# ypw0102/GDR

Measured on AMD Instinct MI355X. Metric: queries/sec on NQ-320k (768-d), higher is better.
Workload: dtype f32; 1 GPU; C2/ragged/prefilter: t5-base encoder 512 q/GPU + Q.D^T top-100, 320000x768 corpus; batch_per_gpu=512, global_batch=512, seq_len=40, corpus_rows=320000, dim=768, k=100, encoder_rows=ragged

## Files before the change

gdr_amd/csrc/sim_topk.hip:

```cpp
#include <stdlib.h>

#include "common.h"

namespace gdr {

constexpr int TILE = 128;
constexpr int SEL_THREADS = 256;

struct SimPlan {
  int64_t tiles_m;
  int stride;
  int64_t n_sample_tiles;
  int64_t n_slots;
  int64_t cap;
  size_t off_val, off_idx, off_cnt, off_thr, off_part, total;
};

static SimPlan make_plan(int B, int64_t N, int k, bool exhaustive, double survivors = 1.0) {
  SimPlan p{};
  p.tiles_m = (N + TILE - 1) / TILE;
  double target = sqrt((double)k * (double)N);
  if (target < k) target = k;
  int64_t ts = (int64_t)((target + TILE - 1) / TILE);
  if (ts < 1) ts = 1;
  if (exhaustive || N <= 16384 || p.tiles_m < 4 * ts) {
    p.stride = 1;
  } else {
    p.stride = (int)(p.tiles_m / ts);
  }
  p.n_sample_tiles = (p.tiles_m + p.stride - 1) / p.stride;
  p.n_slots = p.n_sample_tiles * TILE;
  if (p.stride == 1) {
    p.cap = p.n_slots;
  } else {
    const double n_sample = (double)p.n_slots;
    const double expect = (double)k * (double)N / n_sample;
    p.cap = p.n_slots + (int64_t)(4.0 * expect * survivors) + 4096;
    p.cap = (p.cap + TILE - 1) / TILE * TILE;
  }
  size_t o = 0;
  p.off_val = o, o += align_up((size_t)B * p.cap * sizeof(float), 256);
  p.off_idx = o, o += align_up((size_t)B * p.cap * sizeof(int32_t), 256);
  p.off_cnt = o, o += align_up((size_t)B * CNT_STRIDE * sizeof(int32_t), 256);
  p.off_thr = o, o += align_up((size_t)B * sizeof(float), 256);
  p.off_part = o, o += B <= 32 ? align_up((size_t)B * 16 * 128 * sizeof(unsigned long long), 256) : 0;
  p.total = o;
  return p;
}

__device__ __forceinline__ uint32_t fkey(float v) {
  const uint32_t u = __float_as_uint(v);
  return (u & 0x80000000u) ? ~u : (u | 0x80000000u);
}
__device__ __forceinline__ float fkey_inv(uint32_t k) {
  return __uint_as_float((k & 0x80000000u) ? (k & 0x7fffffffu) : ~k);
}

__device__ __forceinline__ int find_bin(int* hist, int* scan, int& need, int* above, int* res) {
  const int t = threadIdx.x, lane = t & 63, wave = t >> 6;
  const int v = t < 256 ? hist[t] : 0;
  int sfx = v;
#pragma unroll
  for (int off = 1; off < 64; off <<= 1) {
    const int u = __shfl_down(sfx, off);
    if (lane + off < 64) sfx += u;
  }
  if (t < 256 && lane == 0) scan[wave] = sfx;
  if (t == 0) res[0] = 0, res[1] = 0;
  __syncthreads();
  const int w0 = scan[0], w1 = scan[1], w2 = scan[2], w3 = scan[3];
  const int total = w0 + w1 + w2 + w3;
  if (total < need) need = total;
  if (t < 256 && need > 0) {
    const int higher = wave == 0 ? w1 + w2 + w3 : wave == 1 ? w2 + w3 : wave == 2 ? w3 : 0;
    const int mine = sfx + higher, next = mine - v;
    if (mine >= need && next < need) {
      res[0] = t;
      res[1] = next;
    }
  }
  __syncthreads();
  *above = res[1];
  return res[0];
}

__device__ __forceinline__ void wave0_bitonic_desc(unsigned long long* buf, int kpad) {
  if (threadIdx.x >= 64) return;
  const int lane = threadIdx.x;
  for (int size = 2; size <= kpad; size <<= 1) {
    for (int stride = size >> 1; stride > 0; stride >>= 1) {
      for (int t = lane; t < (kpad >> 1); t += 64) {
        const int lo_i = (t / stride) * (stride << 1) + (t % stride), hi_i = lo_i + stride;
        const bool desc = ((lo_i & size) == 0);
        const unsigned long long a = buf[lo_i], b = buf[hi_i];
        if ((a < b) == desc) buf[lo_i] = b, buf[hi_i] = a;
      }
      __builtin_amdgcn_fence(__ATOMIC_RELEASE, "wavefront");
      __builtin_amdgcn_wave_barrier();
      __builtin_amdgcn_fence(__ATOMIC_ACQUIRE, "wavefront");
    }
  }
}

__device__ __forceinline__ void block_minmax(uint32_t& lo, uint32_t& hi, uint32_t* red) {
#pragma unroll
  for (int off = 32; off > 0; off >>= 1) {
    lo = min(lo, (uint32_t)__shfl_xor((int)lo, off));
    hi = max(hi, (uint32_t)__shfl_xor((int)hi, off));
  }
  const int w = threadIdx.x >> 6, nw = blockDim.x >> 6;
  if ((threadIdx.x & 63) == 0) red[w] = lo, red[16 + w] = hi;
  __syncthreads();
  lo = red[0], hi = red[16];
  for (int i = 1; i < nw; ++i) lo = min(lo, red[i]), hi = max(hi, red[16 + i]);
  __syncthreads();
}


__global__ __launch_bounds__(1024) void sim_threshold_kernel(const float* __restrict__ cand_val, int64_t cap,
                                                             int n_slots, int k, float* thr, int32_t* cand_cnt,
                                                             const float* __restrict__ sub) {
  __shared__ int hist[256];
  __shared__ int scan[256];
  __shared__ int res[2];
  __shared__ uint32_t red[32];
  const int q = blockIdx.x;
  const float* v = cand_val + (int64_t)q * cap;
  constexpr int RC = 8;
  const bool cached = n_slots <= RC * (int)blockDim.x;
  uint32_t rk[RC];
#pragma unroll
  for (int u = 0; u < RC; ++u) {
    const int i = threadIdx.x + u * (int)blockDim.x;
    rk[u] = (cached && i < n_slots) ? fkey(v[i]) : 0u;
  }
  const uint32_t kneg = fkey(-INFINITY);
  uint32_t lo = 0xFFFFFFFFu, hi = 0u;
  if (cached) {
#pragma unroll
    for (int u = 0; u < RC; ++u)
      if (rk[u] > kneg) lo = min(lo, rk[u]), hi = max(hi, rk[u]);
  } else {
#pragma unroll 4
    for (int i = threadIdx.x; i < n_slots; i += blockDim.x) {
      const float x = v[i];
      if (x > -INFINITY) {
        const uint32_t key = fkey(x);
        lo = min(lo, key), hi = max(hi, key);
      }
    }
  }
  block_minmax(lo, hi, red);
  if (hi < lo) lo = hi = fkey(-INFINITY);
  const int nbits = hi > lo ? 32 - __clz(hi - lo) : 0;
  const int lsh = 32 - nbits;
  uint32_t prefix = 0;
  int need = k;
  for (int pass = 0; 8 * pass < nbits; ++pass) {
    const int shift = 24 - 8 * pass;
    if (threadIdx.x < 256) hist[threadIdx.x] = 0;
    __syncthreads();
    if (cached) {
#pragma unroll
      for (int u = 0; u < RC; ++u) {
        const uint32_t raw = rk[u];
        const uint32_t key = (raw - lo) << lsh;
        const bool match = pass == 0 ? true : ((key >> (shift + 8)) == (prefix >> (shift + 8)));
        if (raw != 0u && match && raw >= lo) atomicAdd(&hist[(key >> shift) & 255u], 1);
      }
    } else {
#pragma unroll 4
      for (int i = threadIdx.x; i < n_slots; i += blockDim.x) {
        const uint32_t raw = fkey(v[i]);
        const uint32_t key = (raw - lo) << lsh;
        const bool match = pass == 0 ? true : ((key >> (shift + 8)) == (prefix >> (shift + 8)));
        if (match && raw >= lo) atomicAdd(&hist[(key >> shift) & 255u], 1);
      }
    }
    __syncthreads();
    int above;
    const int b = find_bin(hist, scan, need, &above, res);
    need -= above;
    prefix |= (uint32_t)b << shift;
    __syncthreads();
  }
  if (threadIdx.x == 0) {
    const float t = fkey_inv(nbits ? (prefix >> lsh) + lo : lo);
    thr[q] = sub ? t - sub[q] : t;
    cand_cnt[(int64_t)q * CNT_STRIDE] = n_slots;
  }
}

template <bool MERGE>
__global__ __launch_bounds__(1024) void topk_select_kernel(const float* __restrict__ vals,
                                                           const int32_t* __restrict__ idxs,
                                                           const int32_t* __restrict__ cnt, int64_t cap, int G, int B,
                                                           int k, int kpad, int32_t idx_offset,
                                                           const float* __restrict__ thr, float* out_val,
                                                           int32_t* out_idx, int32_t* __restrict__ status, int rs,
                                                           int es) {
  __shared__ int hist[256];
  __shared__ int scan[256];
  __shared__ int res[2];
  __shared__ uint32_t red[32];
  __shared__ int n_out;
  extern __shared__ __attribute__((aligned(16))) unsigned long long sortbuf[];
  const int q = blockIdx.x;
  int count;
  if (MERGE) {
    count = G * k;
    if (status && rs > k && threadIdx.x == 0) {
      int32_t any = 0;
      for (int g = 0; g < G; ++g) any |= idxs[(((int64_t)g * B + q) * rs + k) * es];
      status[q] = any != 0 ? 1 : 0;
    }
  } else {
    const int c = cnt[(int64_t)q * CNT_STRIDE];
    count = c < (int)cap ? c : (int)cap;
    if (status && threadIdx.x == 0) status[q] = c > (int)cap ? 1 : 0;
  }
  auto addr_of = [&](int i) -> int64_t {
    if (MERGE) {
      const int g = i / k, j = i - g * k;
      return (((int64_t)g * B + q) * rs + j) * es;
    }
    return (int64_t)q * cap + i;
  };
  constexpr int RC = 16;
  const bool cached = count <= RC * (int)blockDim.x;
  auto raw_at = [&](int i) -> unsigned long long {
    const int64_t a = addr_of(i);
    const int32_t id = idxs[a];
    if (id < 0) return 0ull;
    return ((unsigned long long)fkey(vals[a]) << 32) | (unsigned long long)(0xFFFFFFFFu - (uint32_t)id);
  };
  unsigned long long rk[RC];
#pragma unroll
  for (int u = 0; u < RC; ++u) {
    const int i = threadIdx.x + u * (int)blockDim.x;
    rk[u] = (cached && i < count) ? raw_at(i) : 0ull;
  }
  uint32_t lo = 0xFFFFFFFFu, hi = 0u;
  if (cached) {
#pragma unroll
    for (int u = 0; u < RC; ++u)
      if (rk[u] != 0ull) {
        const uint32_t key = (uint32_t)(rk[u] >> 32);
        lo = min(lo, key), hi = max(hi, key);
      }
  } else {
#pragma unroll 4
    for (int i = threadIdx.x; i < count; i += blockDim.x) {
      const unsigned long long raw = raw_at(i);
      if (raw != 0ull) {
        const uint32_t key = (uint32_t)(raw >> 32);
        lo = min(lo, key), hi = max(hi, key);
      }
    }
  }
  block_minmax(lo, hi, red);
  if (!MERGE && thr) lo = max(lo, fkey(thr[q]));
  if (hi < lo) hi = lo;
  const int nbits = hi > lo ? 32 - __clz(hi - lo) : 0;
  const int lsh = 32 - nbits;
  auto norm = [&](unsigned long long raw) -> unsigned long long {
    if (raw == 0ull) return 0ull;
    const uint32_t sk = (uint32_t)(raw >> 32);
    if (sk < lo) return 0ull;
    return ((((unsigned long long)(sk - lo)) << 32) | (raw & 0xFFFFFFFFull)) << lsh;
  };
  unsigned long long prefix = 0ull;
  int need = k < count ? k : count;
  int want = need;
  bool exact = false;
  for (int pass = 0; pass < 8 && !exact; ++pass) {
    const int shift = 56 - 8 * pass;
    if (threadIdx.x < 256) hist[threadIdx.x] = 0;
    __syncthreads();
    if (cached) {
#pragma unroll
      for (int u = 0; u < RC; ++u) {
        const unsigned long long key = norm(rk[u]);
        const bool match = pass == 0 ? true : ((key >> (shift + 8)) == (prefix >> (shift + 8)));
        if (match && key != 0ull) atomicAdd(&hist[(int)((key >> shift) & 255ull)], 1);
      }
    } else {
#pragma unroll 4
      for (int i = threadIdx.x; i < count; i += blockDim.x) {
        const unsigned long long key = norm(raw_at(i));
        const bool match = pass == 0 ? true : ((key >> (shift + 8)) == (prefix >> (shift + 8)));
        if (match && key != 0ull) atomicAdd(&hist[(int)((key >> shift) & 255ull)], 1);
      }
    }
    __syncthreads();
    int above;
    const int b = find_bin(hist, scan, need, &above, res);
    if (pass == 0) want = need;
    need -= above;
    prefix |= (unsigned long long)b << shift;
    exact = hist[b] == need;
    __syncthreads();
  }
  if (threadIdx.x == 0) n_out = 0;
  for (int i = threadIdx.x; i < kpad; i += blockDim.x) sortbuf[i] = 0ull;
  __syncthreads();
  if (cached) {
#pragma unroll
    for (int u = 0; u < RC; ++u) {
      const unsigned long long key = norm(rk[u]);
      if (key >= prefix && key != 0ull) {
        const int p = atomicAdd(&n_out, 1);
        if (p < kpad) sortbuf[p] = rk[u];
      }
    }
  } else {
#pragma unroll 4
    for (int i = threadIdx.x; i < count; i += blockDim.x) {
      const unsigned long long raw = raw_at(i);
      const unsigned long long key = norm(raw);
      if (key >= prefix && key != 0ull) {
        const int p = atomicAdd(&n_out, 1);
        if (p < kpad) sortbuf[p] = raw;
      }
    }
  }
  __syncthreads();
  wave0_bitonic_desc(sortbuf, kpad);
  __syncthreads();
  for (int i = threadIdx.x; i < k; i += blockDim.x) {
    const unsigned long long key = sortbuf[i];
    float v = -INFINITY;
    int32_t id = -1;
    if (i < want && key != 0ull) {
      v = fkey_inv((uint32_t)(key >> 32));
      id = (int32_t)(0xFFFFFFFFu - (uint32_t)(key & 0xFFFFFFFFull)) + idx_offset;
    }
    out_val[(int64_t)q * k + i] = v;
    out_idx[(int64_t)q * k + i] = id;
  }
}

constexpr int SL_THREADS = 256, SL_RC = 8, SL_NS_MAX = 16, SL_KPAD_MAX = 128;
struct SelLds {
  int hist[256];
  int scan[256];
  int res[2];
  uint32_t red[32];
  int n_out, last;
};

template <int RC>
__device__ __forceinline__ int block_select_keys(const unsigned long long (&rk)[RC], int k, int kpad, uint32_t lo_floor, SelLds& L,
                                                 unsigned long long* outbuf) {
  uint32_t lo = 0xFFFFFFFFu, hi = 0u;
#pragma unroll
  for (int u = 0; u < RC; ++u)
    if (rk[u] != 0ull) {
      const uint32_t key = (uint32_t)(rk[u] >> 32);
      lo = min(lo, key), hi = max(hi, key);
    }
  block_minmax(lo, hi, L.red);
  lo = max(lo, lo_floor);
  if (hi < lo) hi = lo;
  const int nbits = hi > lo ? 32 - __clz(hi - lo) : 0;
  const int lsh = 32 - nbits;
  auto norm = [&](unsigned long long raw) -> unsigned long long {
    if (raw == 0ull) return 0ull;
    const uint32_t sk = (uint32_t)(raw >> 32);
    if (sk < lo) return 0ull;
    return ((((unsigned long long)(sk - lo)) << 32) | (raw & 0xFFFFFFFFull)) << lsh;
  };
  unsigned long long prefix = 0ull;
  int need = k, want = k;
  bool exact = false;
  for (int pass = 0; pass < 8 && !exact; ++pass) {
    const int shift = 56 - 8 * pass;
    L.hist[threadIdx.x] = 0;
    __syncthreads();
#pragma unroll
    for (int u = 0; u < RC; ++u) {
      const unsigned long long key = norm(rk[u]);
      const bool match = pass == 0 ? true : ((key >> (shift + 8)) == (prefix >> (shift + 8)));
      if (match && key != 0ull) atomicAdd(&L.hist[(int)((key >> shift) & 255ull)], 1);
    }
    __syncthreads();
    int above;
    const int b = find_bin(L.hist, L.scan, need, &above, L.res);
    if (pass == 0) want = need;
    need -= above;
    prefix |= (unsigned long long)b << shift;
    exact = L.hist[b] == need;
    __syncthreads();
  }
  if (threadIdx.x == 0) L.n_out = 0;
  for (int i = threadIdx.x; i < kpad; i += SL_THREADS) outbuf[i] = 0ull;
  __syncthreads();
  if (want > 0) {
#pragma unroll
    for (int u = 0; u < RC; ++u) {
      const unsigned long long key = norm(rk[u]);
      if (key >= prefix && key != 0ull) {
        const int p = atomicAdd(&L.n_out, 1);
        if (p < kpad) outbuf[p] = rk[u];
      }
    }
  }
  __syncthreads();
  return want;
}

struct SlicedArgs {
  const float* vals;
  const int32_t* idxs;
  int32_t* cnt;
  int64_t cap;
  int n_slots;
  int k, kpad, NS;
  int32_t idx_offset;
  float* thr;
  const float* sub;
  unsigned long long* part;
  float* out_val;
  int32_t* out_idx;
  int32_t* status;
};

template <bool THR>
__global__ __launch_bounds__(SL_THREADS) void sim_sliced_select_kernel(const SlicedArgs a) {
  __shared__ SelLds L;
  __shared__ __attribute__((aligned(16))) unsigned long long outbuf[SL_KPAD_MAX];
  const int q = blockIdx.x / a.NS, s = blockIdx.x % a.NS, tid = threadIdx.x;
  int count;
  if (THR) {
    count = a.n_slots;
  } else {
    const int c = a.cnt[(int64_t)q * CNT_STRIDE];
    count = c < (int)a.cap ? c : (int)a.cap;
  }
  const int per = (count + a.NS - 1) / a.NS;
  const int i0 = s * per, i1 = min(count, i0 + per);
  const float* v = a.vals + (int64_t)q * a.cap;
  const int32_t* ix = a.idxs + (int64_t)q * a.cap;
  unsigned long long rk[SL_RC];
#pragma unroll
  for (int u = 0; u < SL_RC; ++u) {
    const int i = i0 + tid + u * SL_THREADS;
    unsigned long long raw = 0ull;
    if (i < i1) {
      const float x = v[i];
      if (THR) {
        if (x > -INFINITY) raw = ((unsigned long long)fkey(x) << 32) | (unsigned long long)(0xFFFFFFFFu - (uint32_t)i);
      } else {
        const int32_t id = ix[i];
        if (id >= 0) raw = ((unsigned long long)fkey(x) << 32) | (unsigned long long)(0xFFFFFFFFu - (uint32_t)id);
      }
    }
    rk[u] = raw;
  }
  const uint32_t floor_key = (!THR && a.thr) ? fkey(a.thr[q]) : 0u;
  block_select_keys<SL_RC>(rk, a.k, a.kpad, floor_key, L, outbuf);
  unsigned long long* mine = a.part + ((int64_t)q * a.NS + s) * a.kpad;
  if (tid < a.kpad) {
    const unsigned long long key = outbuf[tid];
    typedef unsigned int u32x2 __attribute__((ext_vector_type(2)));
    u32x2 w;
    w[0] = (unsigned int)(key & 0xFFFFFFFFull), w[1] = (unsigned int)(key >> 32);
    const __amdgpu_buffer_rsrc_t dst = __builtin_amdgcn_make_buffer_rsrc(mine, 0, a.kpad * 8, 0x00020000);
    __builtin_amdgcn_raw_buffer_store_b64(w, dst, tid * 8, 0, 16);
  }
  asm volatile("s_waitcnt vmcnt(0)" ::: "memory");
  __syncthreads();
  int32_t* ticket = a.cnt + (int64_t)q * CNT_STRIDE + (THR ? 1 : 2);
  if (tid == 0) {
    const int t = __hip_atomic_fetch_add(ticket, 1, __ATOMIC_RELAXED, __HIP_MEMORY_SCOPE_AGENT);
    L.last = t == a.NS - 1;
    if (L.last) {
      __builtin_amdgcn_fence(__ATOMIC_ACQUIRE, "agent");
      asm volatile("s_waitcnt vmcnt(0)" ::: "memory");
    }
  }
  __syncthreads();
  if (!L.last) return;
  const unsigned long long* all = a.part + (int64_t)q * a.NS * a.kpad;
  const int n_all = a.NS * a.kpad;
#pragma unroll
  for (int u = 0; u < SL_RC; ++u) {
    const int i = tid + u * SL_THREADS;
    rk[u] = i < n_all ? all[i] : 0ull;
  }
  const int want = block_select_keys<SL_RC>(rk, a.k, a.kpad, 0u, L, outbuf);
  if (THR) {
    unsigned long long m = tid < want ? outbuf[tid] : ~0ull;
#pragma unroll
    for (int off = 32; off > 0; off >>= 1) {
      const unsigned long long o = __shfl_xor(m, off);
      m = o < m ? o : m;
    }
    if ((tid & 63) == 0) reinterpret_cast<unsigned long long*>(L.hist)[tid >> 6] = m;
    __syncthreads();
    if (tid == 0) {
      const unsigned long long* w4 = reinterpret_cast<const unsigned long long*>(L.hist);
      unsigned long long mm = w4[0];
      for (int i = 1; i < SL_THREADS / 64; ++i) mm = w4[i] < mm ? w4[i] : mm;
      const float t = want > 0 ? fkey_inv((uint32_t)(mm >> 32)) : -INFINITY;
      a.thr[q] = a.sub ? t - a.sub[q] : t;
      a.cnt[(int64_t)q * CNT_STRIDE] = a.n_slots;
      a.cnt[(int64_t)q * CNT_STRIDE + 1] = 0;
      a.cnt[(int64_t)q * CNT_STRIDE + 2] = 0;
    }
    return;
  }
  wave0_bitonic_desc(outbuf, a.kpad);
  __syncthreads();
  for (int i = tid; i < a.k; i += SL_THREADS) {
    const unsigned long long key = outbuf[i];
    float val = -INFINITY;
    int32_t id = -1;
    if (i < want && key != 0ull) {
      val = fkey_inv((uint32_t)(key >> 32));
      id = (int32_t)(0xFFFFFFFFu - (uint32_t)(key & 0xFFFFFFFFull)) + a.idx_offset;
    }
    a.out_val[(int64_t)q * a.k + i] = val;
    a.out_idx[(int64_t)q * a.k + i] = id;
  }
  if (tid == 0) {
    const int c = a.cnt[(int64_t)q * CNT_STRIDE];
    if (a.status) a.status[q] = c > (int)a.cap ? 1 : 0;
    a.cnt[(int64_t)q * CNT_STRIDE + 2] = 0;
  }
}

static int sliced_ns(int64_t len, int kpad) {
  if (kpad > SL_KPAD_MAX || len > (int64_t)SL_NS_MAX * SL_RC * SL_THREADS) return 0;
  int ns = (int)((len + 1023) / 1024);
  const int need = (int)((len + SL_RC * SL_THREADS - 1) / (SL_RC * SL_THREADS));
  if (ns < need) ns = need;
  if (ns < 1) ns = 1;
  if (ns > SL_NS_MAX) ns = SL_NS_MAX;
  while ((int64_t)ns * kpad > SL_RC * SL_THREADS) --ns;
  return ns >= need ? ns : 0;
}

static int next_pow2(int x) {
  int p = 1;
  while (p < x) p <<= 1;
  return p;
}

}

extern "C" size_t gdr_sim_topk_workspace_bytes(int B, int64_t N, int d, int k, int flags) {
  (void)d;
  if (B <= 0 || N <= 0 || k <= 0) return 0;
  return gdr::make_plan(B, N, k, (flags & GDR_SIM_EXHAUSTIVE) != 0).total;
}

namespace gdr {
__global__ __launch_bounds__(256) void cast_f32_bf16_kernel(const float4* __restrict__ in, uint2* __restrict__ out,
                                                            int64_t n4) {
  const int64_t i = (int64_t)blockIdx.x * 256 + threadIdx.x;
  if (i >= n4) return;
  const float4 v = in[i];
  union {
    __bf16 h[4];
    uint2 u;
  } o;
  o.h[0] = (__bf16)v.x, o.h[1] = (__bf16)v.y, o.h[2] = (__bf16)v.z, o.h[3] = (__bf16)v.w;
  out[i] = o.u;
}

static int sim_topk_impl(const void* Q, int B, const void* D, int64_t N, int d, int k, int32_t idx_offset, float* out_val,
                         int32_t* out_idx, int32_t* status, int flags, void* workspace, size_t workspace_bytes,
                         bool bf16, hipStream_t stream);
}

namespace gdr {
int launch_cast_f32_bf16(const float* in, void* out_bf16, int64_t n, hipStream_t stream) {
  if (n == 0) return GDR_OK;
  GDR_CHECK_ARG(in && out_bf16 && n >= 0 && n % 4 == 0, "cast: null pointer or n %% 4 != 0");
  GDR_CHECK_ARG(((uintptr_t)in & 15) == 0 && ((uintptr_t)out_bf16 & 7) == 0, "cast: misaligned pointer");
  if (n == 0) return GDR_OK;
  hipLaunchKernelGGL(cast_f32_bf16_kernel, dim3((unsigned)((n / 4 + 255) / 256)), dim3(256), 0, stream,
                     reinterpret_cast<const float4*>(in), reinterpret_cast<uint2*>(out_bf16), n / 4);
  GDR_CHECK_LAUNCH("cast_f32_bf16_kernel");
  return GDR_OK;
}
}

extern "C" int gdr_cast_f32_bf16(const float* in, void* out_bf16, int64_t n, void* stream_) {
  return gdr::launch_cast_f32_bf16(in, out_bf16, n, static_cast<hipStream_t>(stream_));
}

extern "C" int gdr_sim_topk(const float* Q, int B, const float* D, int64_t N, int d, int k, int32_t idx_offset,
                            float* out_val, int32_t* out_idx, int32_t* status, int flags, void* workspace,
                            size_t workspace_bytes, void* stream_) {
  return gdr::sim_topk_impl(Q, B, D, N, d, k, idx_offset, out_val, out_idx, status, flags, workspace, workspace_bytes,
                            false, static_cast<hipStream_t>(stream_));
}

extern "C" int gdr_sim_topk_bf16(const void* Q, int B, const void* D, int64_t N, int d, int k, int32_t idx_offset,
                                 float* out_val, int32_t* out_idx, int32_t* status, int flags, void* workspace,
                                 size_t workspace_bytes, void* stream_) {
  return gdr::sim_topk_impl(Q, B, D, N, d, k, idx_offset, out_val, out_idx, status, flags, workspace, workspace_bytes,
                            true, static_cast<hipStream_t>(stream_));
}

int gdr::sim_topk_impl(const void* Q, int B, const void* D, int64_t N, int d, int k, int32_t idx_offset,
                       float* out_val, int32_t* out_idx, int32_t* status, int flags, void* workspace,
                       size_t workspace_bytes, bool bf16, hipStream_t stream) {
  if (B == 0) return GDR_OK;
  GDR_CHECK_ARG(Q && D && out_val && out_idx && workspace, "sim_topk: null pointer");
  GDR_CHECK_ARG(B > 0 && N > 0 && d > 0 && d % (bf16 ? 8 : 4) == 0, "sim_topk: bad shape B=%d N=%lld d=%d", B,
                (long long)N, d);
  GDR_CHECK_ARG(k >= 1 && k <= 1024 && k <= N, "sim_topk: k=%d must be in [1, min(1024, N)]", k);
  GDR_CHECK_ARG(N < 0x7fffffffLL - 256, "sim_topk: shard too large for int32 doc ids");
  GDR_CHECK_ARG((int64_t)idx_offset + N <= 0x7fffffffLL,
                "sim_topk: idx_offset=%d + N=%lld leaves int32 doc ids (the largest id, idx_offset + N - 1, must be < 2^31 - 1)", (int)idx_offset,
                (long long)N);
  GDR_CHECK_ARG(((uintptr_t)Q & 15) == 0 && ((uintptr_t)D & 15) == 0 && ((uintptr_t)workspace & 255) == 0,
                "sim_topk: Q, D must be 16-byte and workspace 256-byte aligned");
  const SimPlan p = make_plan(B, N, k, (flags & GDR_SIM_EXHAUSTIVE) != 0);
  if (workspace_bytes < p.total) {
    set_error("sim_topk: workspace %zu < required %zu", workspace_bytes, p.total);
    return GDR_ENOSPC;
  }
  char* ws = static_cast<char*>(workspace);
  SimEpilogue ep{};
  ep.cand_val = reinterpret_cast<float*>(ws + p.off_val);
  ep.cand_idx = reinterpret_cast<int32_t*>(ws + p.off_idx);
  ep.cand_cnt = reinterpret_cast<int32_t*>(ws + p.off_cnt);
  float* thr = reinterpret_cast<float*>(ws + p.off_thr);
  ep.thr = thr;
  ep.status = nullptr;
  ep.cap = (int32_t)p.cap;
  ep.tile_stride = p.stride;
  ep.mode = 1;
  const bool stream_mode = sim_stream_supported(B, d, bf16) && !(flags & GDR_SIM_NO_STREAM);
  int rc = stream_mode ? launch_sim_stream(D, N, Q, B, d, ep, bf16, stream) : launch_sim_gemm(D, N, Q, B, d, ep, bf16, stream);
  if (rc) return rc;
  const int sel_threads = 1024;
  const int kpad = next_pow2(k);
  static const bool sliced_on = [] {
    const char* e = getenv("GDR_SIM_SLICED");
    return e ? atoi(e) != 0 : true;
  }();
  SlicedArgs sa{};
  sa.vals = ep.cand_val, sa.idxs = ep.cand_idx, sa.cnt = ep.cand_cnt, sa.cap = p.cap, sa.n_slots = (int)p.n_slots, sa.k = k, sa.kpad = kpad;
  sa.idx_offset = idx_offset, sa.thr = thr, sa.sub = nullptr, sa.part = reinterpret_cast<unsigned long long*>(ws + p.off_part);
  sa.out_val = out_val, sa.out_idx = out_idx, sa.status = status;
  const int ns_thr = (stream_mode && sliced_on && B <= 32) ? sliced_ns(p.n_slots, kpad) : 0;
  const int ns_sel = (stream_mode && sliced_on && B <= 32) ? sliced_ns(p.cap, kpad) : 0;
  if (ns_thr) {
    sa.NS = ns_thr;
    ProfScope prof(PROF_SELECT, 0.0, stream);
    hipLaunchKernelGGL(sim_sliced_select_kernel<true>, dim3(B * ns_thr), dim3(SL_THREADS), 0, stream, sa);
    GDR_CHECK_LAUNCH("sim_sliced_select_kernel(threshold)");
  } else {
    hipLaunchKernelGGL(sim_threshold_kernel, dim3(B), dim3(sel_threads), 0, stream, ep.cand_val, p.cap, (int)p.n_slots,
                       k, thr, ep.cand_cnt, (const float*)nullptr);
    GDR_CHECK_LAUNCH("sim_threshold_kernel");
  }
  if (p.stride > 1) {
    ep.mode = 2;
    rc = stream_mode ? launch_sim_stream(D, N, Q, B, d, ep, bf16, stream) : launch_sim_gemm(D, N, Q, B, d, ep, bf16, stream);
    if (rc) return rc;
  }
  if (ns_sel) {
    sa.NS = ns_sel;
    ProfScope prof(PROF_SELECT, 0.0, stream);
    hipLaunchKernelGGL(sim_sliced_select_kernel<false>, dim3(B * ns_sel), dim3(SL_THREADS), 0, stream, sa);
    GDR_CHECK_LAUNCH("sim_sliced_select_kernel(select)");
    return GDR_OK;
  }
  hipLaunchKernelGGL(topk_select_kernel<false>, dim3(B), dim3(sel_threads), kpad * sizeof(unsigned long long), stream,
                     ep.cand_val, ep.cand_idx, ep.cand_cnt, p.cap, 1, B, k, kpad, idx_offset, (const float*)thr, out_val,
                     out_idx, status, 0, 1);
  GDR_CHECK_LAUNCH("topk_select_kernel");
  return GDR_OK;
}

namespace gdr {
__global__ __launch_bounds__(256) void sim_qprep_kernel(const float* __restrict__ Q, int d, float dnorm_max, __bf16* __restrict__ Q16,
                                                        float* __restrict__ eps2) {
  __shared__ float red[4];
  const int q = blockIdx.x;
  const float* row = Q + (int64_t)q * d;
  float ss = 0.f;
  for (int c = threadIdx.x * 4; c < d; c += 1024) {
    const float4 v = *reinterpret_cast<const float4*>(row + c);
    ss = fmaf(v.x, v.x, fmaf(v.y, v.y, fmaf(v.z, v.z, fmaf(v.w, v.w, ss))));
    union {
      __bf16 h[4];
      uint2 u;
    } o;
    o.h[0] = (__bf16)v.x, o.h[1] = (__bf16)v.y, o.h[2] = (__bf16)v.z, o.h[3] = (__bf16)v.w;
    *reinterpret_cast<uint2*>(Q16 + (int64_t)q * d + c) = o.u;
  }
#pragma unroll
  for (int off = 32; off > 0; off >>= 1) ss += __shfl_xor(ss, off);
  if ((threadIdx.x & 63) == 0) red[threadIdx.x >> 6] = ss;
  __syncthreads();
  if (threadIdx.x == 0) {
    const float nq = sqrtf(red[0] + red[1] + red[2] + red[3]) * 1.0001f;
    const float c = 0.0078125f + 1.52587890625e-5f + (float)d * 2.384185791015625e-7f;
    eps2[q] = 2.0f * nq * dnorm_max * c * 1.01f;
  }
}

__global__ __launch_bounds__(256) void row_norm2_max_kernel(const float* __restrict__ D, int64_t N, int d, unsigned* __restrict__ out) {
  const int lane = threadIdx.x & 63;
  float best = 0.f;
  for (int64_t r = (int64_t)blockIdx.x * 4 + (threadIdx.x >> 6); r < N; r += (int64_t)gridDim.x * 4) {
    const float* row = D + r * d;
    float ss = 0.f;
    for (int c = lane * 4; c < d; c += 256) {
      const float4 v = *reinterpret_cast<const float4*>(row + c);
      ss = fmaf(v.x, v.x, fmaf(v.y, v.y, fmaf(v.z, v.z, fmaf(v.w, v.w, ss))));
    }
#pragma unroll
    for (int off = 32; off > 0; off >>= 1) ss += __shfl_xor(ss, off);
    best = fmaxf(best, ss);
  }
  if (lane == 0) atomicMax(out, __float_as_uint(best));
}

template <int RC>
__global__ __launch_bounds__(1024) void prefilter_tail_kernel(const float* __restrict__ cand_val, const int32_t* __restrict__ cand_idx,
                                                              const int32_t* __restrict__ cand_cnt, int64_t cap, int k, int cap2,
                                                              int cap2p, const float* __restrict__ eps2, const float* __restrict__ Q,
                                                              const float* __restrict__ D, int d, int32_t idx_offset,
                                                              float* __restrict__ out_val, int32_t* __restrict__ out_idx,
                                                              int32_t* __restrict__ status) {
  __shared__ int hist[256];
  __shared__ int scan[256];
  __shared__ int res[2];
  __shared__ uint32_t red[32];
  __shared__ int n_sh;
  extern __shared__ __attribute__((aligned(16))) unsigned long long pkeys[];
  const int q = blockIdx.x, tid = threadIdx.x, lane = tid & 63, wave = tid >> 6;
  const int c_all = cand_cnt[(int64_t)q * CNT_STRIDE], count = c_all < (int)cap ? c_all : (int)cap;
  const float* v = cand_val + (int64_t)q * cap;
  const int32_t* ix = cand_idx + (int64_t)q * cap;
  const bool cached = count <= RC * 1024;
  uint32_t rk[RC];
#pragma unroll
  for (int u = 0; u < RC; ++u) {
    const int i = tid + u * 1024;
    rk[u] = (cached && i < count) ? fkey(v[i]) : 0u;
  }
  const uint32_t kneg = fkey(-INFINITY);
  uint32_t lo = 0xFFFFFFFFu, hi = 0u;
  if (cached) {
#pragma unroll
    for (int u = 0; u < RC; ++u)
      if (rk[u] > kneg) lo = min(lo, rk[u]), hi = max(hi, rk[u]);
  } else {
    for (int i = tid; i < count; i += 1024) {
      const float x = v[i];
      if (x > -INFINITY) {
        const uint32_t key = fkey(x);
        lo = min(lo, key), hi = max(hi, key);
      }
    }
  }
  block_minmax(lo, hi, red);
  if (hi < lo) lo = hi = fkey(-INFINITY);
  const int nbits = hi > lo ? 32 - __clz(hi - lo) : 0;
  const int lsh = 32 - nbits;
  uint32_t prefix = 0;
  int need = k;
  for (int pass = 0; 8 * pass < nbits; ++pass) {
    const int shift = 24 - 8 * pass;
    if (tid < 256) hist[tid] = 0;
    __syncthreads();
    if (cached) {
#pragma unroll
      for (int u = 0; u < RC; ++u) {
        const uint32_t raw = rk[u];
        const uint32_t key = (raw - lo) << lsh;
        const bool match = pass == 0 ? true : ((key >> (shift + 8)) == (prefix >> (shift + 8)));
        if (raw != 0u && match && raw >= lo) atomicAdd(&hist[(key >> shift) & 255u], 1);
      }
    } else {
      for (int i = tid; i < count; i += 1024) {
        const uint32_t raw = fkey(v[i]);
        const uint32_t key = (raw - lo) << lsh;
        const bool match = pass == 0 ? true : ((key >> (shift + 8)) == (prefix >> (shift + 8)));
        if (match && raw >= lo) atomicAdd(&hist[(key >> shift) & 255u], 1);
      }
    }
    __syncthreads();
    int above;
    const int b = find_bin(hist, scan, need, &above, res);
    need -= above;
    prefix |= (uint32_t)b << shift;
    __syncthreads();
  }
  const float band = fkey_inv(nbits ? (prefix >> lsh) + lo : lo) - eps2[q];
  int32_t* ids = reinterpret_cast<int32_t*>(pkeys + cap2p / 2);
  if (tid == 0) n_sh = 0;
  __syncthreads();
  if (cached) {
#pragma unroll
    for (int u = 0; u < RC; ++u) {
      const int i = tid + u * 1024;
      if (rk[u] > kneg && fkey_inv(rk[u]) >= band) {
        const int32_t id = ix[i];
        if (id >= 0) {
          const int p = atomicAdd(&n_sh, 1);
          if (p < cap2) ids[p] = id;
        }
      }
    }
  } else {
    for (int i = tid; i < count; i += 1024) {
      const int32_t id = ix[i];
      if (id >= 0 && v[i] >= band) {
        const int p = atomicAdd(&n_sh, 1);
        if (p < cap2) ids[p] = id;
      }
    }
  }
  __syncthreads();
  const int n_all = n_sh, n2 = n_all < cap2 ? n_all : cap2;
  if (tid == 0 && status) status[q] = (c_all > (int)cap || n_all > cap2) ? 1 : 0;
  {
    constexpr int MAXP = 4;
    float4 qr[MAXP];
#pragma unroll
    for (int t = 0; t < MAXP; ++t) {
      const int col = lane * 4 + 256 * t;
      qr[t] = col < d ? *reinterpret_cast<const float4*>(Q + (int64_t)q * d + col) : make_float4(0.f, 0.f, 0.f, 0.f);
    }
    float* vals = reinterpret_cast<float*>(pkeys);
    for (int i0 = wave * 2; i0 < n2; i0 += 32) {
      const int i1 = i0 + 1 < n2 ? i0 + 1 : i0;
      const int64_t r0 = ids[i0], r1 = ids[i1];
      float4 a0[MAXP], a1[MAXP];
#pragma unroll
      for (int t = 0; t < MAXP; ++t) {
        const int col = lane * 4 + 256 * t;
        a0[t] = col < d ? *reinterpret_cast<const float4*>(D + r0 * d + col) : make_float4(0.f, 0.f, 0.f, 0.f);
        a1[t] = col < d ? *reinterpret_cast<const float4*>(D + r1 * d + col) : make_float4(0.f, 0.f, 0.f, 0.f);
      }
      float s0 = 0.f, s1 = 0.f;
#pragma unroll
      for (int t = 0; t < MAXP; ++t) {
        s0 = fmaf(qr[t].x, a0[t].x, s0), s0 = fmaf(qr[t].y, a0[t].y, s0), s0 = fmaf(qr[t].z, a0[t].z, s0), s0 = fmaf(qr[t].w, a0[t].w, s0);
        s1 = fmaf(qr[t].x, a1[t].x, s1), s1 = fmaf(qr[t].y, a1[t].y, s1), s1 = fmaf(qr[t].z, a1[t].z, s1), s1 = fmaf(qr[t].w, a1[t].w, s1);
      }
#pragma unroll
      for (int off = 32; off > 0; off >>= 1) s0 += __shfl_xor(s0, off), s1 += __shfl_xor(s1, off);
      if (lane == 0) {
        vals[i0] = s0;
        if (i1 != i0) vals[i1] = s1;
      }
    }
    __syncthreads();
    unsigned long long mykey[4];
#pragma unroll
    for (int u = 0; u < 4; ++u) {
      const int i = tid + u * 1024;
      mykey[u] = 0ull;
      if (i < n2) mykey[u] = ((unsigned long long)fkey(vals[i]) << 32) | (unsigned long long)(0xFFFFFFFFu - (uint32_t)ids[i]);
    }
    __syncthreads();
#pragma unroll
    for (int u = 0; u < 4; ++u) {
      const int i = tid + u * 1024;
      if (i < cap2p) pkeys[i] = mykey[u];
    }
    __syncthreads();
  }
  for (int size = 2; size <= cap2p; size <<= 1) {
    for (int stride = size >> 1; stride > 0; stride >>= 1) {
      for (int t = tid; t < (cap2p >> 1); t += 1024) {
        const int lo_i = (t / stride) * (stride << 1) + (t % stride), hi_i = lo_i + stride;
        const bool desc = ((lo_i & size) == 0);
        const unsigned long long a = pkeys[lo_i], b = pkeys[hi_i];
        if ((a < b) == desc) pkeys[lo_i] = b, pkeys[hi_i] = a;
      }
      __syncthreads();
    }
  }
  for (int i = tid; i < k; i += 1024) {
    const unsigned long long key = pkeys[i];
    float val = -INFINITY;
    int32_t id = -1;
    if (i < n2 && key != 0ull) {
      val = fkey_inv((uint32_t)(key >> 32));
      id = (int32_t)(0xFFFFFFFFu - (uint32_t)(key & 0xFFFFFFFFull)) + idx_offset;
    }
    out_val[(int64_t)q * k + i] = val;
    out_idx[(int64_t)q * k + i] = id;
  }
}

static int prefilter_cap2(int k) {
  int c = 1024;
  while (c < 4 * k) c <<= 1;
  return c;
}
struct PrefilterPlan {
  SimPlan p;
  int cap2;
  size_t off_q16, off_eps, total;
};
static double prefilter_survivor_factor(int64_t N, int d, int k) {
  const SimPlan p0 = make_plan(1, N, k, false);
  if (p0.stride == 1) return 1.0;
  const auto Qf = [](double z) { return 0.5 * erfc(z * 0.70710678118654752); };
  const double tail = (double)k / (double)p0.n_slots;
  double lo = -8.0, hi = 8.0;
  for (int it = 0; it < 60; ++it) {
    const double mid = 0.5 * (lo + hi);
    (Qf(mid) > tail ? lo : hi) = mid;
  }
  const double zl = 0.5 * (lo + hi);
  const double dz = 2.0 * sqrt((double)d) * (0x1p-7 + 0x1p-16 + d * 0x1p-22) * 1.25;
  const double f = 0.5 * Qf(zl - dz) / tail;
  return f > 1.0 ? f : 1.0;
}
static PrefilterPlan make_prefilter_plan(int B, int64_t N, int d, int k) {
  PrefilterPlan pp{};
  pp.p = make_plan(B, N, k, false, prefilter_survivor_factor(N, d, k));
  pp.cap2 = prefilter_cap2(k);
  size_t o = pp.p.total;
  pp.off_q16 = o, o += align_up((size_t)B * d * 2, 256);
  pp.off_eps = o, o += align_up((size_t)B * 4, 256);
  pp.total = o;
  return pp;
}
}

extern "C" size_t gdr_sim_topk_prefilter_workspace_bytes(int B, int64_t N, int d, int k) {
  if (B <= 0 || N <= 0 || k <= 0 || d <= 0) return 0;
  return gdr::make_prefilter_plan(B, N, d, k).total;
}

extern "C" int gdr_row_norm2_max(const float* D, int64_t N, int d, float* out_dev, void* stream_) {
  using namespace gdr;
  hipStream_t stream = static_cast<hipStream_t>(stream_);
  GDR_CHECK_ARG(D && out_dev && N > 0 && d > 0 && d % 4 == 0 && ((uintptr_t)D & 15) == 0, "row_norm2_max: bad arguments");
  if (hipMemsetAsync(out_dev, 0, 4, stream) != hipSuccess) {
    set_error("row_norm2_max: memset failed");
    return GDR_EHIP;
  }
  const int64_t blocks = (N + 3) / 4;
  hipLaunchKernelGGL(row_norm2_max_kernel, dim3((unsigned)(blocks < 4096 ? blocks : 4096)), dim3(256), 0, stream, D, N, d,
                     reinterpret_cast<unsigned*>(out_dev));
  GDR_CHECK_LAUNCH("row_norm2_max_kernel");
  return GDR_OK;
}

extern "C" int gdr_sim_topk_prefilter(const float* Q, int B, const float* D, const void* D_bf16, float dnorm_max, int64_t N, int d, int k,
                                      int32_t idx_offset, float* out_val, int32_t* out_idx, int32_t* status, void* workspace,
                                      size_t workspace_bytes, void* stream_) {
  using namespace gdr;
  hipStream_t stream = static_cast<hipStream_t>(stream_);
  if (B == 0) return GDR_OK;
  GDR_CHECK_ARG(Q && D && D_bf16 && out_val && out_idx && workspace, "sim_topk_prefilter: null pointer");
  GDR_CHECK_ARG(B > 0 && N > 0 && d > 0 && d % 8 == 0 && d <= 1024, "sim_topk_prefilter: bad shape B=%d N=%lld d=%d (d %% 8 == 0, d <= 1024)", B,
                (long long)N, d);
  GDR_CHECK_ARG(k >= 1 && k <= 1024 && k <= N, "sim_topk_prefilter: k=%d must be in [1, min(1024, N)]", k);
  GDR_CHECK_ARG(N < 0x7fffffffLL - 256, "sim_topk_prefilter: shard too large for int32 doc ids");
  GDR_CHECK_ARG((int64_t)idx_offset + N <= 0x7fffffffLL,
                "sim_topk_prefilter: idx_offset=%d + N=%lld leaves int32 doc ids (the largest id, idx_offset + N - 1, must be < 2^31 - 1)",
                (int)idx_offset, (long long)N);
  GDR_CHECK_ARG(dnorm_max > 0.f && dnorm_max < INFINITY, "sim_topk_prefilter: dnorm_max must be the largest row norm of D (> 0, finite)");
  GDR_CHECK_ARG(((uintptr_t)Q & 15) == 0 && ((uintptr_t)D & 15) == 0 && ((uintptr_t)D_bf16 & 15) == 0 && ((uintptr_t)workspace & 255) == 0,
                "sim_topk_prefilter: Q, D, D_bf16 must be 16-byte and workspace 256-byte aligned");
  const PrefilterPlan pp = make_prefilter_plan(B, N, d, k);
  const SimPlan& p = pp.p;
  if (workspace_bytes < pp.total) {
    set_error("sim_topk_prefilter: workspace %zu < required %zu", workspace_bytes, pp.total);
    return GDR_ENOSPC;
  }
  char* ws = static_cast<char*>(workspace);
  SimEpilogue ep{};
  ep.cand_val = reinterpret_cast<float*>(ws + p.off_val);
  ep.cand_idx = reinterpret_cast<int32_t*>(ws + p.off_idx);
  ep.cand_cnt = reinterpret_cast<int32_t*>(ws + p.off_cnt);
  float* thr = reinterpret_cast<float*>(ws + p.off_thr);
  ep.thr = thr, ep.status = nullptr, ep.cap = (int32_t)p.cap, ep.tile_stride = p.stride, ep.mode = 1;
  __bf16* Q16 = reinterpret_cast<__bf16*>(ws + pp.off_q16);
  float* eps2 = reinterpret_cast<float*>(ws + pp.off_eps);
  hipLaunchKernelGGL(sim_qprep_kernel, dim3(B), dim3(256), 0, stream, Q, d, dnorm_max, Q16, eps2);
  GDR_CHECK_LAUNCH("sim_qprep_kernel");
  const bool stream_mode = sim_stream_supported(B, d, true);
  int rc = stream_mode ? launch_sim_stream(D_bf16, N, Q16, B, d, ep, true, stream) : launch_sim_gemm(D_bf16, N, Q16, B, d, ep, true, stream);
  if (rc) return rc;
  hipLaunchKernelGGL(sim_threshold_kernel, dim3(B), dim3(1024), 0, stream, ep.cand_val, p.cap, (int)p.n_slots, k, thr, ep.cand_cnt,
                     (const float*)eps2);
  GDR_CHECK_LAUNCH("sim_threshold_kernel");
  if (p.stride > 1) {
    ep.mode = 2;
    rc = stream_mode ? launch_sim_stream(D_bf16, N, Q16, B, d, ep, true, stream) : launch_sim_gemm(D_bf16, N, Q16, B, d, ep, true, stream);
    if (rc) return rc;
  }
  int cap2p = 1024;
  while (cap2p < pp.cap2) cap2p <<= 1;
  if (int rc__ = ensure_dyn_lds(reinterpret_cast<const void*>(prefilter_tail_kernel<16>), cap2p * 8, "sim_topk_prefilter")) return rc__;
  hipLaunchKernelGGL(prefilter_tail_kernel<16>, dim3(B), dim3(1024), (size_t)cap2p * 8, stream, (const float*)ep.cand_val,
                     (const int32_t*)ep.cand_idx, (const int32_t*)ep.cand_cnt, p.cap, k, pp.cap2, cap2p, (const float*)eps2, Q, D, d,
                     idx_offset, out_val, out_idx, status);
  GDR_CHECK_LAUNCH("prefilter_tail_kernel");
  return GDR_OK;
}

extern "C" int gdr_topk_merge(const float* vals, const int32_t* idx, int G, int B, int k, float* out_val,
                              int32_t* out_idx, void* stream_) {
  using namespace gdr;
  hipStream_t stream = static_cast<hipStream_t>(stream_);
  if (B == 0) return GDR_OK;
  GDR_CHECK_ARG(vals && idx && out_val && out_idx, "topk_merge: null pointer");
  GDR_CHECK_ARG(G > 0 && B > 0 && k >= 1 && k <= 1024, "topk_merge: bad shape G=%d B=%d k=%d", G, B, k);
  const int kpad = next_pow2(k);
  hipLaunchKernelGGL(topk_select_kernel<true>, dim3(B), dim3(SEL_THREADS), kpad * sizeof(unsigned long long), stream,
                     vals, idx, (const int32_t*)nullptr, (int64_t)0, G, B, k, kpad, 0, (const float*)nullptr, out_val, out_idx,
                     (int32_t*)nullptr, k, 1);
  GDR_CHECK_LAUNCH("topk_select_kernel<merge>");
  return GDR_OK;
}

namespace gdr {
__global__ void topk_pack_kernel(const float* __restrict__ vals, const int32_t* __restrict__ idx,
                                 const int32_t* __restrict__ status, int B, int k, int2* __restrict__ pairs) {
  const int64_t e = (int64_t)blockIdx.x * blockDim.x + threadIdx.x;
  if (e >= (int64_t)B * (k + 1)) return;
  const int q = (int)(e / (k + 1)), j = (int)(e - (int64_t)q * (k + 1));
  int2 o;
  if (j < k) {
    o.x = __float_as_int(vals[(int64_t)q * k + j]);
    o.y = idx[(int64_t)q * k + j];
  } else {
    o.x = 0;
    o.y = status ? status[q] : 0;
  }
  pairs[e] = o;
}
}

extern "C" int gdr_topk_pack(const float* vals, const int32_t* idx, const int32_t* status, int B, int k, void* pairs,
                             void* stream_) {
  using namespace gdr;
  hipStream_t stream = static_cast<hipStream_t>(stream_);
  if (B == 0) return GDR_OK;
  GDR_CHECK_ARG(vals && idx && pairs, "topk_pack: null pointer");
  GDR_CHECK_ARG(B > 0 && k >= 1 && k <= 1024, "topk_pack: bad shape B=%d k=%d", B, k);
  const int64_t n = (int64_t)B * (k + 1);
  hipLaunchKernelGGL(topk_pack_kernel, dim3((unsigned)((n + 255) / 256)), dim3(256), 0, stream, vals, idx, status, B, k,
                     static_cast<int2*>(pairs));
  GDR_CHECK_LAUNCH("topk_pack_kernel");
  return GDR_OK;
}

extern "C" int gdr_topk_merge_packed(const void* pairs, int G, int B, int k, float* out_val, int32_t* out_idx,
                                     int32_t* out_status, void* stream_) {
  using namespace gdr;
  hipStream_t stream = static_cast<hipStream_t>(stream_);
  if (B == 0) return GDR_OK;
  GDR_CHECK_ARG(pairs && out_val && out_idx, "topk_merge_packed: null pointer");
  GDR_CHECK_ARG(G > 0 && B > 0 && k >= 1 && k <= 1024, "topk_merge_packed: bad shape G=%d B=%d k=%d", G, B, k);
  const int kpad = next_pow2(k);
  const float* vals = static_cast<const float*>(pairs);
  const int32_t* idx = static_cast<const int32_t*>(pairs) + 1;
  hipLaunchKernelGGL(topk_select_kernel<true>, dim3(B), dim3(SEL_THREADS), kpad * sizeof(unsigned long long), stream,
                     vals, idx, (const int32_t*)nullptr, (int64_t)0, G, B, k, kpad, 0, (const float*)nullptr, out_val, out_idx,
                     out_status, k + 1, 2);
  GDR_CHECK_LAUNCH("topk_select_kernel<merge packed>");
  return GDR_OK;
}
```

Measured before the change: 31260 queries/s.

## Add two-step exact rescoring in prefilter tail with tighter bf16 error bound

```diff
diff --git a/gdr_amd/csrc/sim_topk.hip b/gdr_amd/csrc/sim_topk.hip
--- a/gdr_amd/csrc/sim_topk.hip
+++ b/gdr_amd/csrc/sim_topk.hip
@@ -681,11 +681,11 @@
 
 namespace gdr {
 __global__ __launch_bounds__(256) void sim_qprep_kernel(const float* __restrict__ Q, int d, float dnorm_max, __bf16* __restrict__ Q16,
-                                                        float* __restrict__ eps2) {
-  __shared__ float red[4];
+                                                        float* __restrict__ eps2, int two_step) {
+  __shared__ float red[3][4];
   const int q = blockIdx.x;
   const float* row = Q + (int64_t)q * d;
-  float ss = 0.f;
+  float ss = 0.f, st = 0.f, se = 0.f;
   for (int c = threadIdx.x * 4; c < d; c += 1024) {
     const float4 v = *reinterpret_cast<const float4*>(row + c);
     ss = fmaf(v.x, v.x, fmaf(v.y, v.y, fmaf(v.z, v.z, fmaf(v.w, v.w, ss))));
@@ -695,15 +695,26 @@
     } o;
     o.h[0] = (__bf16)v.x, o.h[1] = (__bf16)v.y, o.h[2] = (__bf16)v.z, o.h[3] = (__bf16)v.w;
     *reinterpret_cast<uint2*>(Q16 + (int64_t)q * d + c) = o.u;
-  }
-#pragma unroll
-  for (int off = 32; off > 0; off >>= 1) ss += __shfl_xor(ss, off);
-  if ((threadIdx.x & 63) == 0) red[threadIdx.x >> 6] = ss;
+    const float tx = (float)o.h[0], ty = (float)o.h[1], tz = (float)o.h[2], tw = (float)o.h[3];
+    st = fmaf(tx, tx, fmaf(ty, ty, fmaf(tz, tz, fmaf(tw, tw, st))));
+    const float ex = tx - v.x, ey = ty - v.y, ez = tz - v.z, ew = tw - v.w;
+    se = fmaf(ex, ex, fmaf(ey, ey, fmaf(ez, ez, fmaf(ew, ew, se))));
+  }
+#pragma unroll
+  for (int off = 32; off > 0; off >>= 1) ss += __shfl_xor(ss, off), st += __shfl_xor(st, off), se += __shfl_xor(se, off);
+  if ((threadIdx.x & 63) == 0) red[0][threadIdx.x >> 6] = ss, red[1][threadIdx.x >> 6] = st, red[2][threadIdx.x >> 6] = se;
   __syncthreads();
   if (threadIdx.x == 0) {
-    const float nq = sqrtf(red[0] + red[1] + red[2] + red[3]) * 1.0001f;
+    const float nq = sqrtf(red[0][0] + red[0][1] + red[0][2] + red[0][3]) * 1.0001f;
     const float c = 0.0078125f + 1.52587890625e-5f + (float)d * 2.384185791015625e-7f;
-    eps2[q] = 2.0f * nq * dnorm_max * c * 1.01f;
+    float eps = nq * dnorm_max * c * 1.01f;
+    if (two_step) {
+      const float nt = sqrtf(red[1][0] + red[1][1] + red[1][2] + red[1][3]) * 1.0001f;
+      const float eq = sqrtf(red[2][0] + red[2][1] + red[2][2] + red[2][3]) * 1.0001f;
+      const float acc = (float)d * 5.9604644775390625e-8f * 1.01f * (nq + 1.00390625f * nt);
+      eps = fminf(eps, dnorm_max * (0.00390625f * nt + eq + acc) * 1.01f);
+    }
+    eps2[q] = 2.0f * eps;
   }
 }
 
@@ -724,18 +735,20 @@
   if (lane == 0) atomicMax(out, __float_as_uint(best));
 }
 
-template <int RC>
+template <int RC, bool TWO>
 __global__ __launch_bounds__(1024) void prefilter_tail_kernel(const float* __restrict__ cand_val, const int32_t* __restrict__ cand_idx,
                                                               const int32_t* __restrict__ cand_cnt, int64_t cap, int k, int cap2,
                                                               int cap2p, const float* __restrict__ eps2, const float* __restrict__ Q,
-                                                              const float* __restrict__ D, int d, int32_t idx_offset,
-                                                              float* __restrict__ out_val, int32_t* __restrict__ out_idx,
-                                                              int32_t* __restrict__ status) {
+                                                              const float* __restrict__ D, int d, float dnorm_max,
+                                                              int32_t idx_offset, float* __restrict__ out_val,
+                                                              int32_t* __restrict__ out_idx, int32_t* __restrict__ status) {
   __shared__ int hist[256];
   __shared__ int scan[256];
   __shared__ int res[2];
   __shared__ uint32_t red[32];
   __shared__ int n_sh;
+  __shared__ float t_sh;
+  __shared__ int nb_sh;
   extern __shared__ __attribute__((aligned(16))) unsigned long long pkeys[];
   const int q = blockIdx.x, tid = threadIdx.x, lane = tid & 63, wave = tid >> 6;
   const int c_all = cand_cnt[(int64_t)q * CNT_STRIDE], count = c_all < (int)cap ? c_all : (int)cap;
@@ -796,68 +809,144 @@
     prefix |= (uint32_t)b << shift;
     __syncthreads();
   }
-  const float band = fkey_inv(nbits ? (prefix >> lsh) + lo : lo) - eps2[q];
+  const float tk = fkey_inv(nbits ? (prefix >> lsh) + lo : lo);
+  constexpr int MAXP = 4;
+  float4 qr[MAXP];
+#pragma unroll
+  for (int t = 0; t < MAXP; ++t) {
+    const int col = lane * 4 + 256 * t;
+    qr[t] = col < d ? *reinterpret_cast<const float4*>(Q + (int64_t)q * d + col) : make_float4(0.f, 0.f, 0.f, 0.f);
+  }
+  const float band = TWO ? tk : tk - eps2[q];
+  float band_old = band;
+  if (TWO) {
+    float part[MAXP];
+#pragma unroll
+    for (int t = 0; t < MAXP; ++t) {
+      float ss = fmaf(qr[t].x, qr[t].x, fmaf(qr[t].y, qr[t].y, fmaf(qr[t].z, qr[t].z, fmaf(qr[t].w, qr[t].w, 0.f))));
+#pragma unroll
+      for (int off = 32; off > 0; off >>= 1) ss += __shfl_xor(ss, off);
+      part[t] = ss;
+    }
+    const float nq = sqrtf(part[0] + part[1] + part[2] + part[3]) * 1.0001f;
+    const float c = 0.0078125f + 1.52587890625e-5f + (float)d * 2.384185791015625e-7f;
+    band_old = tk - 2.0f * (nq * dnorm_max * c * 1.01f);
+  }
   int32_t* ids = reinterpret_cast<int32_t*>(pkeys + cap2p / 2);
-  if (tid == 0) n_sh = 0;
-  __syncthreads();
+  if (tid == 0) n_sh = 0, nb_sh = 0, t_sh = -INFINITY;
+  __syncthreads();
+  int nb = 0;
   if (cached) {
 #pragma unroll
     for (int u = 0; u < RC; ++u) {
       const int i = tid + u * 1024;
-      if (rk[u] > kneg && fkey_inv(rk[u]) >= band) {
+      const float x = fkey_inv(rk[u]);
+      if (rk[u] > kneg && x >= (TWO ? band_old : band)) {
         const int32_t id = ix[i];
         if (id >= 0) {
+          ++nb;
+          if (!TWO || x >= band) {
+            const int p = atomicAdd(&n_sh, 1);
+            if (p < cap2) ids[p] = id;
+          }
+        }
+      }
+    }
+  } else {
+    for (int i = tid; i < count; i += 1024) {
+      const int32_t id = ix[i];
+      const float x = v[i];
+      if (id >= 0 && x >= (TWO ? band_old : band)) {
+        ++nb;
+        if (!TWO || x >= band) {
           const int p = atomicAdd(&n_sh, 1);
           if (p < cap2) ids[p] = id;
         }
       }
     }
-  } else {
-    for (int i = tid; i < count; i += 1024) {
-      const int32_t id = ix[i];
-      if (id >= 0 && v[i] >= band) {
-        const int p = atomicAdd(&n_sh, 1);
-        if (p < cap2) ids[p] = id;
-      }
-    }
-  }
-  __syncthreads();
-  const int n_all = n_sh, n2 = n_all < cap2 ? n_all : cap2;
-  if (tid == 0 && status) status[q] = (c_all > (int)cap || n_all > cap2) ? 1 : 0;
+  }
+  if (TWO && nb) atomicAdd(&nb_sh, nb);
+  __syncthreads();
+  const int n1_all = n_sh, n1 = n1_all < cap2 ? n1_all : cap2;
+  int n_all = n1_all, n2 = n1, sp = cap2p;
+  if (!TWO && tid == 0 && status) status[q] = (c_all > (int)cap || n_all > cap2) ? 1 : 0;
   {
-    constexpr int MAXP = 4;
-    float4 qr[MAXP];
-#pragma unroll
-    for (int t = 0; t < MAXP; ++t) {
-      const int col = lane * 4 + 256 * t;
-      qr[t] = col < d ? *reinterpret_cast<const float4*>(Q + (int64_t)q * d + col) : make_float4(0.f, 0.f, 0.f, 0.f);
-    }
     float* vals = reinterpret_cast<float*>(pkeys);
-    for (int i0 = wave * 2; i0 < n2; i0 += 32) {
-      const int i1 = i0 + 1 < n2 ? i0 + 1 : i0;
-      const int64_t r0 = ids[i0], r1 = ids[i1];
-      float4 a0[MAXP], a1[MAXP];
-#pragma unroll
-      for (int t = 0; t < MAXP; ++t) {
-        const int col = lane * 4 + 256 * t;
-        a0[t] = col < d ? *reinterpret_cast<const float4*>(D + r0 * d + col) : make_float4(0.f, 0.f, 0.f, 0.f);
-        a1[t] = col < d ? *reinterpret_cast<const float4*>(D + r1 * d + col) : make_float4(0.f, 0.f, 0.f, 0.f);
-      }
-      float s0 = 0.f, s1 = 0.f;
-#pragma unroll
-      for (int t = 0; t < MAXP; ++t) {
-        s0 = fmaf(qr[t].x, a0[t].x, s0), s0 = fmaf(qr[t].y, a0[t].y, s0), s0 = fmaf(qr[t].z, a0[t].z, s0), s0 = fmaf(qr[t].w, a0[t].w, s0);
-        s1 = fmaf(qr[t].x, a1[t].x, s1), s1 = fmaf(qr[t].y, a1[t].y, s1), s1 = fmaf(qr[t].z, a1[t].z, s1), s1 = fmaf(qr[t].w, a1[t].w, s1);
-      }
-#pragma unroll
-      for (int off = 32; off > 0; off >>= 1) s0 += __shfl_xor(s0, off), s1 += __shfl_xor(s1, off);
-      if (lane == 0) {
-        vals[i0] = s0;
-        if (i1 != i0) vals[i1] = s1;
-      }
+    const auto score = [&](int begin, int end) {
+      for (int i0 = begin + wave * 2; i0 < end; i0 += 32) {
+        const int i1 = i0 + 1 < end ? i0 + 1 : i0;
+        const int64_t r0 = ids[i0], r1 = ids[i1];
+        float4 a0[MAXP], a1[MAXP];
+#pragma unroll
+        for (int t = 0; t < MAXP; ++t) {
+          const int col = lane * 4 + 256 * t;
+          a0[t] = col < d ? *reinterpret_cast<const float4*>(D + r0 * d + col) : make_float4(0.f, 0.f, 0.f, 0.f);
+          a1[t] = col < d ? *reinterpret_cast<const float4*>(D + r1 * d + col) : make_float4(0.f, 0.f, 0.f, 0.f);
+        }
+        float s0 = 0.f, s1 = 0.f;
+#pragma unroll
+        for (int t = 0; t < MAXP; ++t) {
+          s0 = fmaf(qr[t].x, a0[t].x, s0), s0 = fmaf(qr[t].y, a0[t].y, s0), s0 = fmaf(qr[t].z, a0[t].z, s0), s0 = fmaf(qr[t].w, a0[t].w, s0);
+          s1 = fmaf(qr[t].x, a1[t].x, s1), s1 = fmaf(qr[t].y, a1[t].y, s1), s1 = fmaf(qr[t].z, a1[t].z, s1), s1 = fmaf(qr[t].w, a1[t].w, s1);
+        }
+#pragma unroll
+        for (int off = 32; off > 0; off >>= 1) s0 += __shfl_xor(s0, off), s1 += __shfl_xor(s1, off);
+        if (lane == 0) {
+          vals[i0] = s0;
+          if (i1 != i0) vals[i1] = s1;
+        }
+      }
+    };
+    score(0, n1);
+    if (TWO) {
+      __syncthreads();
+      for (int i = tid; i < n1; i += 1024) {
+        const float x = vals[i];
+        int gt = 0, ge = 0;
+        for (int j = 0; j < n1; j += 4) {
+          const float4 y = *reinterpret_cast<const float4*>(vals + j);
+          gt += y.x > x, ge += y.x >= x;
+          if (j + 1 < n1) gt += y.y > x, ge += y.y >= x;
+          if (j + 2 < n1) gt += y.z > x, ge += y.z >= x;
+          if (j + 3 < n1) gt += y.w > x, ge += y.w >= x;
+        }
+        if (gt < k && ge >= k) t_sh = x;
+      }
+      __syncthreads();
+      const float cut = t_sh - 0.5f * eps2[q];
+      if (cached) {
+#pragma unroll
+        for (int u = 0; u < RC; ++u) {
+          const int i = tid + u * 1024;
+          const float x = fkey_inv(rk[u]);
+          if (rk[u] > kneg && x < tk && x >= cut) {
+            const int32_t id = ix[i];
+            if (id >= 0) {
+              const int p = atomicAdd(&n_sh, 1);
+              if (p < cap2) ids[p] = id;
+            }
+          }
+        }
+      } else {
+        for (int i = tid; i < count; i += 1024) {
+          const float x = v[i];
+          if (x < tk && x >= cut && ix[i] >= 0) {
+            const int p = atomicAdd(&n_sh, 1);
+            if (p < cap2) ids[p] = ix[i];
+          }
+        }
+      }
+      __syncthreads();
+      n_all = n_sh, n2 = n_all < cap2 ? n_all : cap2;
+      if (tid == 0 && status) status[q] = (c_all > (int)cap || n_all > cap2 || nb_sh > cap2) ? 1 : 0;
+      score(n1, n2);
     }
     __syncthreads();
     unsigned long long mykey[4];
+    if (TWO) {
+      sp = 2;
+      while (sp < n2) sp <<= 1;
+    }
 #pragma unroll
     for (int u = 0; u < 4; ++u) {
       const int i = tid + u * 1024;
@@ -868,13 +957,13 @@
 #pragma unroll
     for (int u = 0; u < 4; ++u) {
       const int i = tid + u * 1024;
-      if (i < cap2p) pkeys[i] = mykey[u];
-    }
-    __syncthreads();
-  }
-  for (int size = 2; size <= cap2p; size <<= 1) {
+      if (i < sp) pkeys[i] = mykey[u];
+    }
+    __syncthreads();
+  }
+  for (int size = 2; size <= sp; size <<= 1) {
     for (int stride = size >> 1; stride > 0; stride >>= 1) {
-      for (int t = tid; t < (cap2p >> 1); t += 1024) {
+      for (int t = tid; t < (sp >> 1); t += 1024) {
         const int lo_i = (t / stride) * (stride << 1) + (t % stride), hi_i = lo_i + stride;
         const bool desc = ((lo_i & size) == 0);
         const unsigned long long a = pkeys[lo_i], b = pkeys[hi_i];
@@ -884,10 +973,10 @@
     }
   }
   for (int i = tid; i < k; i += 1024) {
-    const unsigned long long key = pkeys[i];
+    const unsigned long long key = i < n2 ? pkeys[i] : 0ull;
     float val = -INFINITY;
     int32_t id = -1;
-    if (i < n2 && key != 0ull) {
+    if (key != 0ull) {
       val = fkey_inv((uint32_t)(key >> 32));
       id = (int32_t)(0xFFFFFFFFu - (uint32_t)(key & 0xFFFFFFFFull)) + idx_offset;
     }
@@ -985,7 +1074,11 @@
   ep.thr = thr, ep.status = nullptr, ep.cap = (int32_t)p.cap, ep.tile_stride = p.stride, ep.mode = 1;
   __bf16* Q16 = reinterpret_cast<__bf16*>(ws + pp.off_q16);
   float* eps2 = reinterpret_cast<float*>(ws + pp.off_eps);
-  hipLaunchKernelGGL(sim_qprep_kernel, dim3(B), dim3(256), 0, stream, Q, d, dnorm_max, Q16, eps2);
+  static const bool two_step = [] {
+    const char* e = getenv("GDR_SIM_TAIL_TWO_STEP");
+    return e ? atoi(e) != 0 : true;
+  }();
+  hipLaunchKernelGGL(sim_qprep_kernel, dim3(B), dim3(256), 0, stream, Q, d, dnorm_max, Q16, eps2, (int)two_step);
   GDR_CHECK_LAUNCH("sim_qprep_kernel");
   const bool stream_mode = sim_stream_supported(B, d, true);
   int rc = stream_mode ? launch_sim_stream(D_bf16, N, Q16, B, d, ep, true, stream) : launch_sim_gemm(D_bf16, N, Q16, B, d, ep, true, stream);
@@ -1000,10 +1093,11 @@
   }
   int cap2p = 1024;
   while (cap2p < pp.cap2) cap2p <<= 1;
-  if (int rc__ = ensure_dyn_lds(reinterpret_cast<const void*>(prefilter_tail_kernel<16>), cap2p * 8, "sim_topk_prefilter")) return rc__;
-  hipLaunchKernelGGL(prefilter_tail_kernel<16>, dim3(B), dim3(1024), (size_t)cap2p * 8, stream, (const float*)ep.cand_val,
-                     (const int32_t*)ep.cand_idx, (const int32_t*)ep.cand_cnt, p.cap, k, pp.cap2, cap2p, (const float*)eps2, Q, D, d,
-                     idx_offset, out_val, out_idx, status);
+  const auto tail = two_step ? prefilter_tail_kernel<16, true> : prefilter_tail_kernel<16, false>;
+  if (int rc__ = ensure_dyn_lds(reinterpret_cast<const void*>(tail), cap2p * 8, "sim_topk_prefilter")) return rc__;
+  hipLaunchKernelGGL(tail, dim3(B), dim3(1024), (size_t)cap2p * 8, stream, (const float*)ep.cand_val, (const int32_t*)ep.cand_idx,
+                     (const int32_t*)ep.cand_cnt, p.cap, k, pp.cap2, cap2p, (const float*)eps2, Q, D, d, dnorm_max, idx_offset, out_val,
+                     out_idx, status);
   GDR_CHECK_LAUNCH("prefilter_tail_kernel");
   return GDR_OK;
 }
```

Result: no change. 31450 queries/s (median of 6 runs) (+0.6%).
